# jessicabonnie/dandd

Hardware: AMD Instinct MI355X
Metric: Gbp/s sketched over k-sweep (higher is better)
Workload: dtype u64; 1 GPU; cfg2: 10 x 50 Mbp synthetic FASTA on this GPU (10 over 1 GPU(s)) resident in HBM, HLL log2m=14, k-sweep 4-40 (K=37), leaf sketches + root union + all cardinalities + delta; genomes_per_gpu=10, bases_per_genome=50000000, kmin=4, kmax=40, log2m=14, parallelism=genomes sharded over 1 GPU(s)

## Files before the change

### dandd_amd/csrc/dd_sketch_api.hip

```cpp
#include "dd_ctx.h"

static int ensure_side_streams(dd_ctx* c, int n) {
    if (!c->side_go) DD_HIP(hipEventCreateWithFlags(&c->side_go, hipEventDisableTiming));
    for (int i = 0; i < std::min(n, 8); ++i) {
        if (c->side[i]) continue;
        DD_HIP(hipStreamCreateWithFlags(&c->side[i], hipStreamNonBlocking));
        DD_HIP(hipEventCreateWithFlags(&c->side_done[i], hipEventDisableTiming));
    }
    return DD_OK;
}

struct SideLanes {
    dd_ctx* c;
    int lane = 0;
    template <class F>
    int run(bool fork, F&& launch) {
        const int l = lane & 7;
        if (!fork) return launch(c->stream), DD_OK;
        DD_HIP(hipStreamWaitEvent(c->side[l], c->side_go, 0));
        launch(c->side[l]);
        DD_HIP(hipEventRecord(c->side_done[l], c->side[l]));
        DD_HIP(hipStreamWaitEvent(c->stream, c->side_done[l], 0));
        ++lane;
        return DD_OK;
    }
};

struct Bitmaps { uint32_t* small = nullptr; uint32_t* big = nullptr; size_t big_stride = 0; uint32_t* sat = nullptr; };
static int reserve_bitmaps(dd_ctx* c, const dd::PlanKnobs& knobs, const size_t* nbytes, int ngenomes, int kmin, int kmax, size_t sat_words, Bitmaps& bm) {
    int rc, ka = 0, kb = 0;
    if (kmin <= dd::kBitmapMaxK || sat_words) {
        const size_t words = kmin <= dd::kBitmapMaxK ? (size_t)ngenomes * dd::kBitmapStride : 0, bbytes = (words + sat_words) * sizeof(uint32_t);
        if ((rc = c->bitmaps.reserve(bbytes))) return rc;
        if (words) bm.small = static_cast<uint32_t*>(c->bitmaps.p);
        if (sat_words) bm.sat = static_cast<uint32_t*>(c->bitmaps.p) + words;
        DD_HIP(hipMemsetAsync(c->bitmaps.p, 0, bbytes, c->stream));
    }
    if (dd::plan_bigmap_range(c->p, kmin, kmax, knobs, nbytes, ngenomes, &ka, &kb)) {
        bm.big_stride = dd::bigmap_offset_words(kb + 1, c->canonical != 0);
        const size_t bbytes = (size_t)ngenomes * bm.big_stride * sizeof(uint32_t);
        if ((rc = c->bigmaps.reserve(bbytes))) return rc;
        bm.big = static_cast<uint32_t*>(c->bigmaps.p);
        DD_HIP(hipMemsetAsync(bm.big, 0, bbytes, c->stream));
    }
    return DD_OK;
}

static int cached_plan(dd_ctx* c, StageSet& stage, const dd::PlanKnobs& knobs, const size_t* nbytes, int ngenomes, int kmin, int kmax, dd_ctx::PlanEntry** out) {
    dd_ctx::PlanEntry* pc = &c->plans[0];
    for (auto& pe : c->plans) {
        if (pe.valid && pe.kmin == kmin && pe.kmax == kmax && pe.knobs == knobs && pe.sizes.size() == (size_t)ngenomes &&
            std::equal(pe.sizes.begin(), pe.sizes.end(), nbytes)) {
            pe.last_use = ++c->plan_clock;
            *out = &pe;
            return DD_OK;
        }
        if (pe.last_use < pc->last_use) pc = &pe;
    }
    pc->last_use = ++c->plan_clock;
    pc->valid = false;
    pc->classes = dd::plan_sweep(c->p, c->canonical, nbytes, ngenomes, kmin, kmax, knobs);
    size_t job_bytes = 0;
    pc->job_off.assign(pc->classes.size(), 0);
    for (size_t i = 0; i < pc->classes.size(); ++i) {
        pc->job_off[i] = job_bytes;
        job_bytes += align_up(sizeof(dd::SweepJob) * pc->classes[i].jobs.size(), 256);
    }
    int rc;
    if ((rc = pc->jobtab.reserve(job_bytes))) return rc;
    if ((rc = stage.jobs.reserve(job_bytes))) return rc;
    for (size_t i = 0; i < pc->classes.size(); ++i)
        if ((rc = upload(c, stage.jobs, static_cast<char*>(pc->jobtab.p) + pc->job_off[i], pc->classes[i].jobs.data(),
                         sizeof(dd::SweepJob) * pc->classes[i].jobs.size(), pc->job_off[i])))
            return rc;
    pc->kmin = kmin;
    pc->kmax = kmax;
    pc->knobs = knobs;
    pc->sizes.assign(nbytes, nbytes + ngenomes);
    pc->valid = true;
    *out = pc;
    return DD_OK;
}

static int upload_bucket_rows(dd_ctx* c, StageSet& stage, const std::vector<dd::SweepClass>& classes, int ngenomes, int kmin, int kmax, uint8_t* regs_dev,
                              const dd::BucketRow** rows_dev) {
    const dd::BucketLayout lay = dd::bucket_layout(classes, c->p, ngenomes, kmin, kmax);
    if (!lay.total) return DD_OK;
    std::vector<dd::BucketRow> rtab((size_t)ngenomes * lay.K);
    int rc;
    if ((rc = c->buckets.reserve(lay.total))) return rc;
    if ((rc = stage.rows.reserve(lay.cursors - lay.table))) return rc;
    char* bb = static_cast<char*>(c->buckets.p);
    dd::bucket_rows(lay, bb, regs_dev, c->p, ngenomes, rtab.data());
    DD_HIP(hipMemsetAsync(bb + lay.zero_begin, 0, lay.zero_bytes, c->stream));
    if ((rc = upload(c, stage.rows, bb + lay.table, rtab.data(), sizeof(dd::BucketRow) * rtab.size(), 0))) return rc;
    *rows_dev = reinterpret_cast<const dd::BucketRow*>(bb + lay.table);
    return DD_OK;
}

static int ensure_universe(dd_ctx* c, int kfirst, int last_k) {
    if (!last_k) return DD_OK;
    const size_t m = (size_t)1 << c->p;
    int rc;
    if ((rc = c->universe.reserve((size_t)(dd::kSatMaxK - dd::kSatMinK + 1) * m))) return rc;
    for (int k = std::max(kfirst, dd::kSatMinK); k <= last_k; ++k) {
        if (c->universe_built[k - dd::kSatMinK]) continue;
        dd::launch_universe(static_cast<uint8_t*>(c->universe.p) + (size_t)(k - dd::kSatMinK) * m, k, c->p, c->canonical, c->stream);
        DD_HIP(hipGetLastError());
        c->universe_built[k - dd::kSatMinK] = true;
    }
    return DD_OK;
}

static void launch_lds_class(dd_ctx* c, const dd::SweepClass& sc, const dd::SweepGenome* gt, const dd::SweepJob* jt, int ngenomes, int kmin, int sat_last_k, hipStream_t ks) {
    if (sc.kclass == dd::kBitmapClass) {
        dd::launch_bitmap(gt, jt, (int)sc.jobs.size(), sc.kfirst, sc.klast, c->canonical, ks);
        dd::launch_bitmap_finish(gt, ngenomes, sc.kfirst, sc.klast, kmin, c->p, ks);
    } else if (sc.kclass == dd::kBigmapClass) {
        dd::launch_bigmap(gt, jt, (int)sc.jobs.size(), c->canonical, ks);
        dd::launch_bigmap_finish(gt, ngenomes, sc.kfirst, sc.klast, kmin, c->p, c->canonical, ks);
    } else {
        dd::launch_sweep(gt, jt, (int)sc.jobs.size(), sc.kclass, sc.plan, static_cast<const uint8_t*>(c->universe.p), sat_last_k, ks);
    }
}

static int launch_classes(dd_ctx* c, const dd_ctx::PlanEntry& plan, const dd::SweepGenome* gtab, const dd::BucketRow* rows, int ngenomes, int kmin, int kmax, int sat_last_k, int* blocks) {
    const int K = kmax - kmin + 1;
    size_t lds_jobs = 0;
    int lds_classes = 0, nepochs = 0, rc;
    for (const dd::SweepClass& sc : plan.classes) {
        if (sc.plan.mode != dd::kBucketMode) lds_jobs += sc.jobs.size(), ++lds_classes;
        else nepochs = sc.plan.nepochs;
    }
    const bool side = lds_classes > 1 && lds_jobs < 12000, side_b = nepochs > 1;
    if ((side || side_b) && (rc = ensure_side_streams(c, side_b ? (int)plan.classes.size() : lds_classes))) return rc;
    Span phase(c, DD_KERNEL_SWEEP, side || side_b);
    if (side || side_b) DD_HIP(hipEventRecord(c->side_go, c->stream));
    SideLanes lanes{c};
    for (size_t i = 0; i < plan.classes.size(); ++i) {
        const dd::SweepClass& sc = plan.classes[i];
        const dd::SweepJob* jobs = reinterpret_cast<const dd::SweepJob*>(static_cast<char*>(plan.jobtab.p) + plan.job_off[i]);
        const bool bucket = sc.plan.mode == dd::kBucketMode, on_lane = side_b || (side && !bucket);
        rc = lanes.run(on_lane, [&](hipStream_t ks) {
            if (!bucket) {
                Span span(c, DD_KERNEL_SWEEP, !on_lane);
                launch_lds_class(c, sc, gtab, jobs, ngenomes, kmin, sat_last_k, ks);
            }
            const dd::ScatterParams sp{rows, K, sc.plan.logg, sc.plan.cap_chunks, sc.plan.nb_log2};
            for (int e = 0; bucket && e < sc.plan.nepochs; ++e) {
                const size_t j0 = sc.epoch_begin[e], j1 = sc.epoch_begin[e + 1];
                if (j1 == j0) continue;
                Span span(c, DD_KERNEL_SWEEP, !on_lane);
                dd::launch_scatter(gtab, jobs + j0, (int)(j1 - j0), sc.kclass, sc.plan, sp, ks, e == 0);
                dd::launch_replay(rows, ngenomes, K, sc.kfirst - kmin, sc.klast - sc.kfirst + 1, sc.plan, ks, e == 0);
            }
        });
        if (rc) return rc;
        *blocks += (int)sc.jobs.size();
    }
    DD_HIP(hipGetLastError());
    return DD_OK;
}

extern "C" {

int dd_sketch_device(dd_ctx* c, const uint8_t* const* fasta_dev, const size_t* nbytes, int ngenomes,
                     int kmin, int kmax, uint8_t* regs_dev) {
    if (check_ctx(c)) return DD_EINVAL;
    if (ngenomes < 0 || !regs_dev || (ngenomes && (!fasta_dev || !nbytes)))
        return fail(DD_EINVAL, "null argument");
    if (kmin < 1 || kmax > 64 || kmin > kmax) return fail(DD_EINVAL, "k range %d..%d outside 1..64", kmin, kmax);
    uint64_t tokens_ub = 0;
    for (int g = 0; g < ngenomes; ++g) {
        if (nbytes[g] && !fasta_dev[g]) return fail(DD_EINVAL, "genome %d: null buffer", g);
        if (reinterpret_cast<uintptr_t>(fasta_dev[g]) & 15)
            return fail(DD_EINVAL, "genome %d: device buffer must be 16-byte aligned", g);
        tokens_ub += nbytes[g];
    }
    DeviceGuard guard(c->device);
    const size_t K = (size_t)(kmax - kmin + 1), m = (size_t)1 << c->p;
    DD_HIP(hipMemsetAsync(regs_dev, 0, (size_t)ngenomes * K * m, c->stream));
    if (!ngenomes) return DD_OK;

    dd::PlanKnobs knobs = dd::PlanKnobs::from_env();
    if (!getenv("DD_BUCKET_GB")) knobs.bucket_budget = c->bucket_budget;
    std::vector<dd::PackGenome> ptab;
    size_t max_chunks = 0;
    Bitmaps bm;
    int rc;
    if ((rc = layout_tokens(c, fasta_dev, nbytes, ngenomes, ptab, max_chunks))) return rc;
    const int sat_last_k = dd::plan_saturate_last_k(c->p, c->canonical, kmin, kmax, knobs, nbytes, ngenomes);
    if ((rc = reserve_bitmaps(c, knobs, nbytes, ngenomes, kmin, kmax, sat_last_k ? (size_t)ngenomes * K : 0, bm))) return rc;
    if ((rc = ensure_universe(c, kmin, sat_last_k))) return rc;
    std::vector<dd::SweepGenome> gtab(ngenomes);
    for (int g = 0; g < ngenomes; ++g) {
        const dd::TokenStream& ts = ptab[g].out;
        gtab[g] = dd::SweepGenome{ts.codes, ts.bad, ts.ntok, regs_dev + (size_t)g * K * m,
                                  bm.small ? bm.small + (size_t)g * dd::kBitmapStride : nullptr,
                                  bm.big ? bm.big + (size_t)g * bm.big_stride : nullptr,
                                  bm.sat ? bm.sat + (size_t)g * K : nullptr};
    }

    const size_t pack_off = align_up(sizeof(dd::SweepGenome) * ngenomes, 256);
    const size_t gtab_bytes = pack_off + align_up(sizeof(dd::PackGenome) * ngenomes, 256);
    if ((rc = c->tables.reserve(gtab_bytes))) return rc;
    StageSet& stage = c->stage[c->stage_cur ^= 1];
    DD_HIP(hipEventSynchronize(stage.free));
    if ((rc = stage.tables.reserve(gtab_bytes))) return rc;
    char* tdev = static_cast<char*>(c->tables.p);
    if ((rc = upload(c, stage.tables, tdev, gtab.data(), sizeof(dd::SweepGenome) * ngenomes, 0))) return rc;
    if ((rc = upload(c, stage.tables, tdev + pack_off, ptab.data(), sizeof(dd::PackGenome) * ngenomes, pack_off))) return rc;
    {
        Span sp(c, DD_KERNEL_PACK);
        dd::launch_pack_batch(reinterpret_cast<const dd::PackGenome*>(tdev + pack_off), ngenomes, max_chunks, c->stream);
    }
    DD_HIP(hipGetLastError());

    dd_ctx::PlanEntry* plan = nullptr;
    const dd::BucketRow* rows_dev = nullptr;
    int blocks = 0;
    if ((rc = cached_plan(c, stage, knobs, nbytes, ngenomes, kmin, kmax, &plan))) return rc;
    if ((rc = upload_bucket_rows(c, stage, plan->classes, ngenomes, kmin, kmax, regs_dev, &rows_dev))) return rc;
    DD_HIP(hipEventRecord(stage.free, c->stream));
    if ((rc = launch_classes(c, *plan, reinterpret_cast<const dd::SweepGenome*>(tdev), rows_dev, ngenomes, kmin, kmax, sat_last_k, &blocks))) return rc;
    c->st_tokens = tokens_ub;
    c->st_updates = tokens_ub * (uint64_t)K;
    c->st_blocks = blocks;
    return DD_OK;
}

int dd_sketch_buffer(dd_ctx* c, const uint8_t* fasta, size_t nbytes, int kmin, int kmax, uint8_t* regs) {
    if (check_ctx(c)) return DD_EINVAL;
    if (!regs || (nbytes && !fasta)) return fail(DD_EINVAL, "null argument");
    if (kmin < 1 || kmax > 64 || kmin > kmax) return fail(DD_EINVAL, "k range %d..%d outside 1..64", kmin, kmax);
    DeviceGuard guard(c->device);
    const size_t K = (size_t)(kmax - kmin + 1), m = (size_t)1 << c->p;
    int rc;
    dd::FileBuf fq;
    if (dd::has_plus_line(fasta, nbytes)) {
        if (!fq.reserve(nbytes + 16)) return fail(DD_ENOMEM, "out of host memory");
        fq.len = nbytes = dd::fastq_to_fasta(fasta, nbytes, fq.p);
        fasta = fq.p;
    }
    if ((rc = c->fasta.reserve(nbytes + 16))) return rc;
    if ((rc = c->regs.reserve(K * m))) return rc;
    if (nbytes) DD_HIP(hipMemcpyAsync(c->fasta.p, fasta, nbytes, hipMemcpyHostToDevice, c->stream));
    const uint8_t* ptrs[1] = {static_cast<const uint8_t*>(c->fasta.p)};
    const size_t ns[1] = {nbytes};
    if ((rc = dd_sketch_device(c, ptrs, ns, 1, kmin, kmax, static_cast<uint8_t*>(c->regs.p)))) return rc;
    DD_HIP(hipMemcpyAsync(regs, c->regs.p, K * m, hipMemcpyDeviceToHost, c->stream));
    DD_HIP(hipStreamSynchronize(c->stream));
    return DD_OK;
}

}
```

### dandd_amd/csrc/dd_sweep.hip

```cpp
#include "dd_common.h"
#include "dd_kernels.h"
#include "dd_k1.h"

namespace dd {
namespace {

template <int KC, bool CANON, bool CHECK, typename Win>
DD_D void sweep_token(const Win& win, int run, int kfirst, int nk, int p, RaiseQueue& s) {
    constexpr bool QUEUE = KC != 0;
    asm volatile("" : "+s"(nk));
    int j = 0;
#pragma unroll 1
    for (; j + 1 < nk; j += 2) {
        const int k = kfirst + j;
        const bool ok0 = !CHECK || run >= k, ok1 = !CHECK || run > k;
        const unsigned long long okm0 = CHECK ? __builtin_amdgcn_ballot_w64(run >= k) : ~0ull, okm1 = CHECK ? __builtin_amdgcn_ballot_w64(run > k) : ~0ull;
        if (CHECK && !okm0) return;
        sweep_update2<QUEUE, CHECK>(s, (uint32_t)j, win.template hash<CANON>(k), okm0, ok0,
                                    (uint32_t)j + 1u, win.template hash<CANON>(k + 1), okm1, ok1, p);
    }
    if (j < nk) {
        const int k = kfirst + j;
        const unsigned long long okm = CHECK ? __builtin_amdgcn_ballot_w64(run >= k) : ~0ull;
        if (!CHECK || okm) sweep_update<QUEUE, CHECK>(s, (uint32_t)j, win.template hash<CANON>(k), okm, !CHECK || run >= k, p);
    }
}

template <int KC, bool CANON>
__global__ __launch_bounds__(1024) void sweep_kernel(const SweepGenome* __restrict__ genomes,
                                                    const SweepJob* __restrict__ jobs, int p, uint32_t queue_off,
                                                    const uint8_t* __restrict__ universe, int universe_last_k) {
    lds_starts_at_zero();
    const SweepJob job = jobs[blockIdx.x];
    const SweepGenome g = genomes[job.genome];
    int nk = job.nk, kfirst = job.kfirst, krow = job.krow;
    const uint32_t m = 1u << p;

    int nsat = 0;
    if constexpr (KC == 0) {
        if (g.sat && kfirst <= universe_last_k) nsat = min(nk, universe_last_k - kfirst + 1);
        if (nsat) {
            uint32_t* const word = reinterpret_cast<uint32_t*>(g_lds);
            if (threadIdx.x == 0) {
                uint32_t d = 0;
                while (d < (uint32_t)nsat && load4_fresh(g.sat + krow + d)) ++d;
                *word = d;
            }
            __syncthreads();
            const int d = __builtin_amdgcn_readfirstlane((int)*word);
            __syncthreads();
            kfirst += d, nk -= d, krow += d, nsat -= d;
            if (nk == 0) return;
        }
    }
    const unsigned long long ntok = gload8u(g.ntok);
    uint8_t* const slab = g.regs + ((size_t)krow << p);

    TileIn next;
    fetch_tile(g, job, ntok, job.tile_begin, next);

    {
        uint4* z = reinterpret_cast<uint4*>(g_lds);
        const uint32_t n16 = (uint32_t)nk * (m >> 4);
        for (uint32_t i = threadIdx.x; i < n16; i += blockDim.x) z[i] = load16_fresh(slab + (size_t)i * 16);
    }
    __syncthreads();

    const int kmaxg = kfirst + nk - 1;
    RaiseQueue s;
    s.base = queue_off + (uint32_t)__builtin_amdgcn_readfirstlane(threadIdx.x >> 6) * (kRaiseQueueRecords * 4u);
    s.dense = (KC != 0 && queue_off) ? kRaiseDense : 0u;
    s.waiting = 0;

    for (unsigned tile = job.tile_begin; tile < job.tile_end; ++tile) {
        const TileIn cur = next;
        fetch_tile(g, job, ntok, tile + 1, next);
        if (!__any(cur.live)) continue;
        SweepWindows<KC> win;
        walk_segment(cur, win, [&](auto clean, int run) {
            if constexpr (decltype(clean)::value) {
                sweep_token<KC, CANON, false>(win, 0, kfirst, nk, p, s);
            } else {
                if (__all(run >= kmaxg)) sweep_token<KC, CANON, false>(win, run, kfirst, nk, p, s);
                else sweep_token<KC, CANON, true>(win, run, kfirst, nk, p, s);
            }
        });
    }
    if (s.dense) sweep_drain(s);
    __syncthreads();

    const uint4* l4 = reinterpret_cast<const uint4*>(g_lds);
    uint32_t* gw = reinterpret_cast<uint32_t*>(slab);
    const uint32_t n16 = (uint32_t)nk * (m >> 4);
    const uint32_t nsat16 = (uint32_t)nsat * (m >> 4);
    const uint8_t* const urow = universe + ((size_t)(kfirst - kSatMinK) << p);
    uint32_t short_rows = 0;
    for (uint32_t i = threadIdx.x; i < n16; i += blockDim.x) {
        const uint4 lv = l4[i];
        const uint4 gv = load16_fresh(slab + (size_t)i * 16);
        const uint32_t l[4] = {lv.x, lv.y, lv.z, lv.w};
        const uint32_t o[4] = {gv.x, gv.y, gv.z, gv.w};
        uint32_t u[4] = {0u, 0u, 0u, 0u}, below = 0;
        if (KC == 0 && i < nsat16) {
            const uint4 uv = gload16(urow + (size_t)i * 16);
            u[0] = uv.x, u[1] = uv.y, u[2] = uv.z, u[3] = uv.w;
        }
#pragma unroll
        for (int q = 0; q < 4; ++q) {
            uint32_t old = o[q];
            uint32_t mx = bmax4(old, l[q]);
            while (mx != old) {
                uint32_t prev = gcas32(&gw[4 * i + q], old, mx);
                if (prev == old) break;
                old = prev;
                mx = bmax4(old, l[q]);
            }
            below |= mx ^ u[q];
        }
        if (KC == 0 && i < nsat16 && below) short_rows |= 1u << (i >> (p - 4));
    }
    if constexpr (KC == 0) {
        if (nsat) {
            uint32_t* const word = reinterpret_cast<uint32_t*>(g_lds);
            __syncthreads();
            if (threadIdx.x == 0) *word = 0u;
            __syncthreads();
            if (short_rows) atomicOr(word, short_rows);
            __syncthreads();
            if (threadIdx.x < (uint32_t)nsat && !((*word >> threadIdx.x) & 1u)) gor32(g.sat + krow + threadIdx.x, 1u);
        }
    }
}

__constant__ int c_bitmap_off[kBitmapMaxK + 2] = {0, bitmap_offset(1), bitmap_offset(2), bitmap_offset(3),
                                                 bitmap_offset(4), bitmap_offset(5), bitmap_offset(6),
                                                 bitmap_offset(7), bitmap_offset(8), bitmap_offset(9),
                                                 kBitmapWords};
static_assert(kBitmapMaxK == 9 && bitmap_offset(9) + bitmap_words(9) == kBitmapWords &&
              kBitmapWords + kBitmapMaxK < kBitmapStride, "bitmap layout");

template <bool CANON>
__global__ __launch_bounds__(1024) __attribute__((amdgpu_num_sgpr(72))) void bitmap_kernel(const SweepGenome* __restrict__ genomes,
                                                     const SweepJob* __restrict__ jobs) {
    const SweepJob job = jobs[blockIdx.x];
    const SweepGenome g = genomes[job.genome];
    const int kfirst = job.kfirst, klast = job.kfirst + job.nk - 1;
    const unsigned long long ntok = gload8u(g.ntok);
    const int w0 = c_bitmap_off[kfirst], w1 = c_bitmap_off[klast + 1];
    uint32_t* const bits = reinterpret_cast<uint32_t*>(g_lds) - w0;
    uint32_t kmask = __builtin_amdgcn_readfirstlane(((2u << klast) - 1u) & ~((1u << kfirst) - 1u));
    uint32_t* const complete = g.bitmap + kBitmapWords;
    __shared__ uint32_t have[kBitmapMaxK + 2];
    __shared__ uint32_t flagged;
    if (threadIdx.x == 0) {
        uint32_t f = 0;
        for (int k = kfirst; k <= klast; ++k)
            if (load4_fresh(complete + k)) f |= 1u << k;
        flagged = f;
    }
    if (threadIdx.x <= kBitmapMaxK) have[threadIdx.x] = 0;
    __syncthreads();
    kmask = __builtin_amdgcn_readfirstlane(kmask & ~flagged);
    if (kmask == 0u) return;
    for (int i = w0 + (int)threadIdx.x; i < w1; i += blockDim.x) {
        const uint32_t v = load4_fresh(&g.bitmap[i]);
        bits[i] = v;
        if (v) {
            int k = kfirst;
            for (int j = kfirst + 1; j <= klast; ++j) k = (i >= c_bitmap_off[j]) ? j : k;
            atomicAdd(&have[k], (uint32_t)__builtin_popcount(v));
        }
    }
    __syncthreads();
    auto all_of = [](int k) { return CANON ? (1u << (2 * k - 1)) + ((k & 1) ? 0u : (1u << (k - 1))) : (1u << (2 * k)); };
    for (int k = kfirst; k <= klast; ++k) {
        if (have[k] == all_of(k)) {
            kmask &= ~(1u << k);
            if (threadIdx.x == 0) gstore4(complete + k, 1u);
        }
    }
    kmask = __builtin_amdgcn_readfirstlane(kmask);
    if (kmask == 0u) return;

    const int prime = klast - 1;
    for (unsigned tile = job.tile_begin; tile < job.tile_end; ++tile) {
        const unsigned long long seg = (unsigned long long)tile * blockDim.x + threadIdx.x;
        if (seg * kSegTokens >= ntok) continue;
        SmallWindows<true> win{};
        const SmallIn in = fetch_small(g, seg, prime, win);
        const uint4 sc = in.sc;
        const uint2 sb = in.sb;
        int run = in.run;
        const uint32_t cws[4] = {sc.x, sc.y, sc.z, sc.w};
#pragma unroll
        for (int w = 0; w < 4; ++w) {
            const uint32_t bw = ((w & 2) ? sb.y : sb.x) >> ((w & 1) * 16);
#pragma unroll 1
            for (int i = 0; i < 16; ++i) {
                const uint32_t c = (cws[w] >> (2 * i)) & 3u;
                run = ((bw >> i) & 1u) ? 0 : run + 1;
                win.push(c);
                uint32_t xs[kBitmapMaxK + 1], seen[kBitmapMaxK + 1];
                uint32_t all_seen = 1u;
#pragma unroll
                for (int k = 1; k <= kBitmapMaxK; ++k) {
                    if (!((kmask >> k) & 1u)) continue;
                    uint32_t x = win.fw & ((1u << (2 * k)) - 1u);
                    if (CANON) {
                        const uint32_t r = win.rc >> (32 - 2 * k);
                        x = x < r ? x : r;
                    }
                    xs[k] = x;
                    seen[k] = bits[bitmap_offset(k) + (x >> 5)];
                    all_seen &= seen[k] >> (x & 31u);
                }
                if (!(all_seen & 1u)) {
#pragma unroll
                    for (int k = 1; k <= kBitmapMaxK; ++k) {
                        if (!((kmask >> k) & 1u) || run < k) continue;
                        if (!((seen[k] >> (xs[k] & 31u)) & 1u))
                            atomicOr(&bits[bitmap_offset(k) + (xs[k] >> 5)], 1u << (xs[k] & 31u));
                    }
                }
            }
        }
    }
    __syncthreads();
    if (threadIdx.x <= kBitmapMaxK) have[threadIdx.x] = 0;
    __syncthreads();
    for (int i = w0 + (int)threadIdx.x; i < w1; i += blockDim.x) {
        const uint32_t mine = bits[i], theirs = load4_fresh(&g.bitmap[i]);
        if (mine & ~theirs) gor32(&g.bitmap[i], mine);
        int k = kfirst;
        for (int j = kfirst + 1; j <= klast; ++j) k = (i >= c_bitmap_off[j]) ? j : k;
        if (mine | theirs) atomicAdd(&have[k], (uint32_t)__builtin_popcount(mine | theirs));
    }
    __syncthreads();
    if (threadIdx.x >= (unsigned)kfirst && threadIdx.x <= (unsigned)klast && have[threadIdx.x] == all_of((int)threadIdx.x))
        gstore4(complete + threadIdx.x, 1u);
}

__global__ __launch_bounds__(1024) void bitmap_finish_kernel(const SweepGenome* __restrict__ genomes,
                                                            int kfirst, int kmin, int p, int tile_log2) {
    lds_starts_at_zero();
    const SweepGenome g = genomes[blockIdx.y];
    const int k = kfirst + (int)blockIdx.x;
    const uint32_t b = blockIdx.z;
    const uint32_t* bm = g.bitmap + c_bitmap_off[k];
    const uint32_t nw = (uint32_t)(c_bitmap_off[k + 1] - c_bitmap_off[k]);
    uint8_t* const row = g.regs + ((size_t)(k - kmin) << p);
    if (gridDim.z > 1 && nw <= 512) {
        if (b != 0) return;
        for_each_set_bit(bm, nw, [&](uint32_t x) { hll_update(RegsGlobal{row}, wang64_fast<true>(x), p); });
        return;
    }
    finish_tile(row + ((size_t)b << tile_log2), tile_log2, b, p, [&](const auto& emit) { for_each_set_bit(bm, nw, emit); });
}


template <bool CANON>
DD_D uint32_t bigmap_index(uint32_t fw, uint32_t rc, int k) {
    if (!CANON) return fw;
    if (k & 1) {
        const uint32_t y = ((fw >> k) & 1u) ? rc : fw;
        return ((y >> (k + 1)) << k) | (y & ((1u << k) - 1u));
    }
    return fw < rc ? fw : rc;
}
template <bool CANON>
DD_D uint32_t bigmap_kmer(uint32_t idx, int k) {
    if (!CANON || !(k & 1)) return idx;
    const uint32_t y = ((idx >> k) << (k + 1)) | (idx & ((1u << k) - 1u));
    uint32_t r = __brev(y);
    r = ((r >> 1) & 0x55555555u) | ((r & 0x55555555u) << 1);
    r = (~r) >> (32 - 2 * k);
    return y < r ? y : r;
}

template <bool CANON>
__global__ __launch_bounds__(1024) void bigmap_kernel(const SweepGenome* __restrict__ genomes, const SweepJob* __restrict__ jobs) {
    const SweepJob job = jobs[blockIdx.x];
    const SweepGenome g = genomes[job.genome];
    const int k = job.kfirst;
    const uint32_t slice = (uint32_t)job.slice;
    const unsigned long long ntok = gload8u(g.ntok);
    uint32_t* const home = g.bigmap + bigmap_offset_words(k, CANON) + (size_t)slice * kBigmapSliceWords;
    uint32_t* const bits = reinterpret_cast<uint32_t*>(g_lds);
    for (int i = threadIdx.x; i < kBigmapSliceWords; i += blockDim.x) bits[i] = load4_fresh(home + i);
    __syncthreads();
    const uint32_t mask = (1u << (2 * k)) - 1u;
    const int top = 2 * k - 2, prime = k - 1;
    for (unsigned tile = job.tile_begin; tile < job.tile_end; ++tile) {
        const unsigned long long seg = (unsigned long long)tile * blockDim.x + threadIdx.x;
        if (seg * kSegTokens >= ntok) continue;
        SmallWindows<false> win{mask, top};
        const SmallIn in = fetch_small(g, seg, prime, win);
        const uint4 sc = in.sc;
        const uint2 sb = in.sb;
        int run = in.run;
        const uint32_t cws[4] = {sc.x, sc.y, sc.z, sc.w};
        auto record = [&](uint32_t idx, bool ok) {
            if ((idx >> 20) == slice && ok) {
                const uint32_t at = (idx & 0xFFFFFu) >> 5, bit = 1u << (idx & 31u);
                if (!(bits[at] & bit)) atomicOr(&bits[at], bit);
            }
        };
        if (__all((sb.x | sb.y) == 0u && run >= prime)) {
#pragma unroll
            for (int w = 0; w < 4; ++w) {
#pragma unroll 4
                for (int i = 0; i < 16; ++i) {
                    const uint32_t c = (cws[w] >> (2 * i)) & 3u;
                    win.push(c);
                    record(bigmap_index<CANON>(win.fw, win.rc, k), true);
                }
            }
            continue;
        }
#pragma unroll
        for (int w = 0; w < 4; ++w) {
            const uint32_t bw = ((w & 2) ? sb.y : sb.x) >> ((w & 1) * 16);
#pragma unroll 4
            for (int i = 0; i < 16; ++i) {
                const uint32_t c = (cws[w] >> (2 * i)) & 3u;
                run = ((bw >> i) & 1u) ? 0 : run + 1;
                win.push(c);
                record(bigmap_index<CANON>(win.fw, win.rc, k), run >= k);
            }
        }
    }
    __syncthreads();
    for (int i = threadIdx.x; i < kBigmapSliceWords; i += blockDim.x) {
        const uint32_t mine = bits[i];
        if (mine && (mine & ~load4_fresh(home + i))) gor32(home + i, mine);
    }
}

template <bool CANON>
__global__ __launch_bounds__(1024) void bigmap_finish_kernel(const SweepGenome* __restrict__ genomes,
                                                            int kfirst, int kmin, int p, int tile_log2) {
    lds_starts_at_zero();
    const SweepGenome g = genomes[blockIdx.y];
    const int k = kfirst + (int)blockIdx.x;
    const uint32_t b = blockIdx.z;
    const uint32_t* bm = g.bigmap + bigmap_offset_words(k, CANON);
    const uint32_t nw = (uint32_t)bigmap_slices(k, CANON) * kBigmapSliceWords;
    finish_tile(g.regs + ((size_t)(k - kmin) << p) + ((size_t)b << tile_log2), tile_log2, b, p, [&](const auto& emit) {
        for_each_set_bit(bm, nw, [&](uint32_t idx) { emit(bigmap_kmer<CANON>(idx, k)); });
    });
}

template <bool CANON>
__global__ __launch_bounds__(1024) void universe_kernel(uint8_t* __restrict__ row, int k, int p) {
    lds_starts_at_zero();
    const uint32_t m = 1u << p;
    uint4* z = reinterpret_cast<uint4*>(g_lds);
    for (uint32_t i = threadIdx.x; i < (m >> 4); i += blockDim.x) z[i] = make_uint4(0, 0, 0, 0);
    __syncthreads();
    const uint32_t n = 1u << (2 * k);
    for (uint32_t x = blockIdx.x * blockDim.x + threadIdx.x; x < n; x += gridDim.x * blockDim.x) {
        if (CANON) {
            uint32_t r = __brev(x);
            r = ((r >> 1) & 0x55555555u) | ((r & 0x55555555u) << 1);
            r = (~r) >> (32 - 2 * k);
            if (r < x) continue;
        }
        const Probe q = probe(wang64_fast<true>(x), p);
        lds_raise(q.hi >> (32 - p), rho_of(q, p));
    }
    __syncthreads();
    const uint4* l4 = reinterpret_cast<const uint4*>(g_lds);
    uint32_t* gw = reinterpret_cast<uint32_t*>(row);
    for (uint32_t i = threadIdx.x; i < (m >> 4); i += blockDim.x) {
        const uint4 lv = l4[i];
        const uint4 gv = load16_fresh(row + (size_t)i * 16);
        const uint32_t l[4] = {lv.x, lv.y, lv.z, lv.w};
        const uint32_t o[4] = {gv.x, gv.y, gv.z, gv.w};
#pragma unroll
        for (int q = 0; q < 4; ++q) {
            uint32_t old = o[q];
            uint32_t mx = bmax4(old, l[q]);
            while (mx != old) {
                uint32_t prev = gcas32(&gw[4 * i + q], old, mx);
                if (prev == old) break;
                old = prev;
                mx = bmax4(old, l[q]);
            }
        }
    }
}

}

void launch_universe(uint8_t* row_dev, int k, int log2m, int canonical, hipStream_t st) {
    if (k < kSatMinK || k > kSatMaxK || log2m < 4 || log2m > 16) return;
    (void)hipMemsetAsync(row_dev, 0, (size_t)1 << log2m, st);
    const unsigned grid = std::min(1024u, 1u << (2 * k - 16));
    dispatch_bool(canonical != 0, [&](auto cn) {
        hipLaunchKernelGGL(universe_kernel<decltype(cn)::value>, dim3(grid), dim3(1024), (size_t)1 << log2m, st, row_dev, k, log2m);
    });
}

int sweep_max_lds_bytes() { return 160 * 1024; }

void launch_bitmap(const SweepGenome* genomes, const SweepJob* jobs, int njobs, int kfirst, int klast,
                   int canonical, hipStream_t st) {
    if (njobs <= 0 || kfirst < 1 || klast > kBitmapMaxK || klast < kfirst) return;
    const size_t lds = (size_t)(bitmap_offset(klast) + bitmap_words(klast) - bitmap_offset(kfirst)) * 4;
    dispatch_bool(canonical != 0, [&](auto cn) {
        launch_full_lds<bitmap_kernel<decltype(cn)::value>, 256>(dim3((unsigned)njobs), dim3(1024), lds, st, genomes, jobs);
    });
}

void launch_bitmap_finish(const SweepGenome* genomes, int ngenomes, int kfirst, int klast, int kmin, int log2m,
                          hipStream_t st) {
    if (ngenomes <= 0 || klast < kfirst) return;
    const int tile_log2 = std::min(log2m, 16);
    hipLaunchKernelGGL(bitmap_finish_kernel, dim3((unsigned)(klast - kfirst + 1), (unsigned)ngenomes, 1u << (log2m - tile_log2)), dim3(1024),
                       (size_t)1 << tile_log2, st, genomes, kfirst, kmin, log2m, tile_log2);
}

void launch_bigmap(const SweepGenome* genomes, const SweepJob* jobs, int njobs, int canonical, hipStream_t st) {
    if (njobs <= 0) return;
    dispatch_bool(canonical != 0, [&](auto cn) {
        launch_full_lds<bigmap_kernel<decltype(cn)::value>>(dim3((unsigned)njobs), dim3(1024), (size_t)kBigmapSliceWords * 4, st, genomes, jobs);
    });
}

void launch_bigmap_finish(const SweepGenome* genomes, int ngenomes, int kfirst, int klast, int kmin, int log2m,
                          int canonical, hipStream_t st) {
    if (ngenomes <= 0 || klast < kfirst) return;
    const int tile_log2 = std::min(log2m, 17);
    const dim3 grid((unsigned)(klast - kfirst + 1), (unsigned)ngenomes, 1u << (log2m - tile_log2));
    dispatch_bool(canonical != 0, [&](auto cn) {
        launch_full_lds<bigmap_finish_kernel<decltype(cn)::value>>(grid, dim3(1024), (size_t)1 << tile_log2, st, genomes, kfirst, kmin, log2m, tile_log2);
    });
}

void launch_sweep(const SweepGenome* genomes, const SweepJob* jobs, int njobs, int kclass,
                  const SweepPlan& plan, const uint8_t* universe, int universe_last_k, hipStream_t st) {
    if (njobs <= 0) return;
    if (!universe || kclass != 0) universe_last_k = 0;
    dispatch_kc_canon(kclass, plan.canonical, [&](auto kc, auto cn) {
        launch_full_lds<sweep_kernel<decltype(kc)::value, decltype(cn)::value>>(dim3((unsigned)njobs), dim3((unsigned)plan.threads), (size_t)plan.lds_bytes, st,
                                                                                genomes, jobs, plan.log2m, (uint32_t)plan.queue_off, universe, universe_last_k);
    });
}

}
```

Baseline: 38.93 Gbp/s.

## Overlap small-k bitmap class on side stream with hashed sweep classes

Adds a side_k mode: when there are no bucket classes, a small-k bitmap class exists alongside hashed LDS classes, and precision is low, the bitmap class is forked onto a side stream. It is joined only after all classes are launched, so it runs concurrently with the hashed sweep kernels. SideLanes is changed to support deferred joins. The bitmap kernel also replaces a serial single-thread loop over completion flags with a wavefront-parallel load plus ballot. The overlap risks contention for compute units and shared memory, and it disables per-kernel timing spans in this mode.

Result: faster. 39.62 Gbp/s, median of 6 (+1.8%).

```diff
diff --git a/dandd_amd/csrc/dd_sketch_api.hip b/dandd_amd/csrc/dd_sketch_api.hip
--- a/dandd_amd/csrc/dd_sketch_api.hip
+++ b/dandd_amd/csrc/dd_sketch_api.hip
@@ -12,16 +12,21 @@
 
 struct SideLanes {
     dd_ctx* c;
-    int lane = 0;
+    int lane = 0, joined = 0;
     template <class F>
-    int run(bool fork, F&& launch) {
+    int run(bool fork, F&& launch, bool join_now = true) {
         const int l = lane & 7;
         if (!fork) return launch(c->stream), DD_OK;
-        DD_HIP(hipStreamWaitEvent(c->side[l], c->side_go, 0));
-        launch(c->side[l]);
-        DD_HIP(hipEventRecord(c->side_done[l], c->side[l]));
-        DD_HIP(hipStreamWaitEvent(c->stream, c->side_done[l], 0));
+        const hipError_t waited = hipStreamWaitEvent(c->side[l], c->side_go, 0);
+        if (waited == hipSuccess) launch(c->side[l]);
+        const hipError_t marked = hipEventRecord(c->side_done[l], c->side[l]);
         ++lane;
+        DD_HIP(waited);
+        DD_HIP(marked);
+        return join_now ? join() : DD_OK;
+    }
+    int join() {
+        for (; joined < lane; ++joined) DD_HIP(hipStreamWaitEvent(c->stream, c->side_done[joined & 7], 0));
         return DD_OK;
     }
 };
@@ -126,38 +131,47 @@
 
 static int launch_classes(dd_ctx* c, const dd_ctx::PlanEntry& plan, const dd::SweepGenome* gtab, const dd::BucketRow* rows, int ngenomes, int kmin, int kmax, int sat_last_k, int* blocks) {
     const int K = kmax - kmin + 1;
-    size_t lds_jobs = 0;
-    int lds_classes = 0, nepochs = 0, rc;
+    size_t lds_jobs = 0, side_jobs = 12000;
+    int lds_classes = 0, hashed_lds = 0, nbucket = 0, nepochs = 0, rc;
+    bool small_k = false;
     for (const dd::SweepClass& sc : plan.classes) {
         if (sc.plan.mode != dd::kBucketMode) lds_jobs += sc.jobs.size(), ++lds_classes;
-        else nepochs = sc.plan.nepochs;
-    }
-    const bool side = lds_classes > 1 && lds_jobs < 12000, side_b = nepochs > 1;
-    if ((side || side_b) && (rc = ensure_side_streams(c, side_b ? (int)plan.classes.size() : lds_classes))) return rc;
-    Span phase(c, DD_KERNEL_SWEEP, side || side_b);
-    if (side || side_b) DD_HIP(hipEventRecord(c->side_go, c->stream));
+        else nepochs = sc.plan.nepochs, ++nbucket;
+        if (sc.kclass == dd::kBitmapClass) small_k = true;
+        else if (sc.kclass >= 0 && sc.plan.mode != dd::kBucketMode) ++hashed_lds;
+    }
+    if (const char* s = getenv("DD_SIDE_JOBS")) side_jobs = (size_t)strtoull(s, nullptr, 10);
+    const bool side = lds_classes > 1 && lds_jobs < side_jobs, side_b = nepochs > 1;
+    const bool side_k = !side && !side_b && !nbucket && small_k && hashed_lds && c->p <= 16 && !getenv("DD_NO_SIDE_SMALLK");
+    const bool forks = side || side_b || side_k;
+    if (forks && (rc = ensure_side_streams(c, side_b ? (int)plan.classes.size() : side_k ? 1 : lds_classes))) return rc;
+    Span phase(c, DD_KERNEL_SWEEP, forks);
+    if (forks) DD_HIP(hipEventRecord(c->side_go, c->stream));
     SideLanes lanes{c};
     for (size_t i = 0; i < plan.classes.size(); ++i) {
         const dd::SweepClass& sc = plan.classes[i];
         const dd::SweepJob* jobs = reinterpret_cast<const dd::SweepJob*>(static_cast<char*>(plan.jobtab.p) + plan.job_off[i]);
-        const bool bucket = sc.plan.mode == dd::kBucketMode, on_lane = side_b || (side && !bucket);
+        const bool bucket = sc.plan.mode == dd::kBucketMode;
+        const bool on_lane = side_b || (side && !bucket) || (side_k && sc.kclass == dd::kBitmapClass), timed = !on_lane && !side_k;
         rc = lanes.run(on_lane, [&](hipStream_t ks) {
             if (!bucket) {
-                Span span(c, DD_KERNEL_SWEEP, !on_lane);
+                Span span(c, DD_KERNEL_SWEEP, timed);
                 launch_lds_class(c, sc, gtab, jobs, ngenomes, kmin, sat_last_k, ks);
             }
             const dd::ScatterParams sp{rows, K, sc.plan.logg, sc.plan.cap_chunks, sc.plan.nb_log2};
             for (int e = 0; bucket && e < sc.plan.nepochs; ++e) {
                 const size_t j0 = sc.epoch_begin[e], j1 = sc.epoch_begin[e + 1];
                 if (j1 == j0) continue;
-                Span span(c, DD_KERNEL_SWEEP, !on_lane);
+                Span span(c, DD_KERNEL_SWEEP, timed);
                 dd::launch_scatter(gtab, jobs + j0, (int)(j1 - j0), sc.kclass, sc.plan, sp, ks, e == 0);
                 dd::launch_replay(rows, ngenomes, K, sc.kfirst - kmin, sc.klast - sc.kfirst + 1, sc.plan, ks, e == 0);
             }
-        });
-        if (rc) return rc;
+        }, !side_k);
+        if (rc) break;
         *blocks += (int)sc.jobs.size();
     }
+    const int jrc = lanes.join();
+    if (rc || jrc) return rc ? rc : jrc;
     DD_HIP(hipGetLastError());
     return DD_OK;
 }
diff --git a/dandd_amd/csrc/dd_sweep.hip b/dandd_amd/csrc/dd_sweep.hip
--- a/dandd_amd/csrc/dd_sweep.hip
+++ b/dandd_amd/csrc/dd_sweep.hip
@@ -152,11 +152,11 @@
     uint32_t* const complete = g.bitmap + kBitmapWords;
     __shared__ uint32_t have[kBitmapMaxK + 2];
     __shared__ uint32_t flagged;
-    if (threadIdx.x == 0) {
-        uint32_t f = 0;
-        for (int k = kfirst; k <= klast; ++k)
-            if (load4_fresh(complete + k)) f |= 1u << k;
-        flagged = f;
+    if (threadIdx.x < 64) {
+        const int k = (int)threadIdx.x;
+        const uint32_t v = (k >= kfirst && k <= klast) ? load4_fresh(complete + k) : 0u;
+        const unsigned long long f = __ballot(v != 0u);
+        if (threadIdx.x == 0) flagged = (uint32_t)f;
     }
     if (threadIdx.x <= kBitmapMaxK) have[threadIdx.x] = 0;
     __syncthreads();
```
